# medivhna/TF_Face_Toolbox

Hardware: AMD Instinct MI355X
Metric: images/sec (whole node), SphereFaceNet-20 112x112 bs512 (higher is better)
Workload: dtype f32; 1 GPU; SphereFaceNet-20 + A-softmax training step, 112x112x3, global batch 512, 10575 classes, Momentum, fp32; global_batch=512, per_gpu_batch=512, parallelism=dp1

## Files before the change

### tf_face_toolbox_amd/csrc/api.hip

```cpp
#include <hip/hip_runtime.h>
#include <stdio.h>
#include <stdlib.h>
#include <string.h>

#include <initializer_list>

#include "../../include/fte.h"
#include "conv_plan.h"
#include "igemm.h"
#include "wgrad16.h"
#include "pw16.h"
#include "kernels.h"
#include "layers.h"
#include "wino.h"
#include "search.h"
#include "partial_fc.h"
#include "cluster.h"
#include "iresnet.h"

namespace {

inline int rc(hipError_t e) { return e == hipSuccess ? FTE_OK : (int)e; }

const PlanKnobs& knobs() {
    static const PlanKnobs k = plan_knobs_from_env();
    return k;
}
const Planner& planner(PlanCtx c, int epi) {
    if (c.bf16 || c.bn) {
        static const Planner host = {knobs(), {}};
        return host;
    }
    auto with_device = [](int e) {
        Planner p = {knobs(), {}};
        p.d.cus = igemm_num_cus();
        const int tile = sk_tile(p.k, e);
        for (int t : {tile, tile == TILE_128x128 ? (int)TILE_128x64 : tile})
            if (t >= 0 && t < 5) p.d.sk_bpc[t][e] = igemm_sk_blocks_per_cu(t, e);
        return p;
    };
    if (epi == EPI_FWD) {
        static const Planner fwd = with_device(EPI_FWD);
        return fwd;
    }
    static const Planner dgrad = with_device(EPI_DGRAD);
    return dgrad;
}
inline PlanCtx ctx32(bool bn = false) { return {igemm_get_bf16(), false, bn, wino_get_algo()}; }
inline PlanCtx ctx16(bool s16, bool bn = false) { return {true, s16, bn, wino_get_algo()}; }
template <class F>
size_t max_over_modes(bool bn, F total) {
    size_t need = 0;
    const int algo = wino_get_algo();
    for (const PlanCtx& c : {PlanCtx{false, false, bn, algo}, PlanCtx{true, false, bn, algo}, PlanCtx{true, true, bn, algo}}) {
        const size_t v = total(c);
        if (v > need) need = v;
    }
    return need;
}

inline void zero_params(IgemmParams* p) { memset(p, 0, sizeof(*p)); }

inline void plain_a(IgemmParams* p, const float* a, int ld, int kc) {
    p->A = a; p->a_OH = 1; p->a_OW = 1; p->a_IH = 1; p->a_IW = 1; p->a_stride = 1;
    p->a_ld = ld; p->a_KC = kc; p->a_NT = 1;
}
inline void conv_taps(IgemmParams* p, int ksize, const Pads& ph, const Pads& pw) {
    p->a_NT = ksize * ksize;
    for (int r = 0; r < ksize; ++r)
        for (int s = 0; s < ksize; ++s) { p->a_dh[r * ksize + s] = r - ph.before; p->a_dw[r * ksize + s] = s - pw.before; }
}

inline bool set_bytes(IgemmParams* p, size_t a_elems, size_t b_elems, size_t esize = 4) {
    const size_t lim = (size_t)1 << 31;
    if (a_elems * esize >= lim || b_elems * esize >= lim) return false;
    p->a_bytes = (unsigned)(a_elems * esize);
    p->b_bytes = (unsigned)(b_elems * esize);
    return true;
}

inline hipError_t launch_rows(IgemmParams p, const RowPlan& rp, int al, int bl, int epi, long prow0, float* pw, hipStream_t st) {
    const int M = p.M;
    hipError_t e = hipSuccess;
    if (rp.tail_mode == 3) {
        int bm, bn;
        igemm_tile_dims(rp.main_tile, &bm, &bn);
        const long T = rp.main_mtiles * (p.N / bn), iters = T * (p.K / 32);
        p.m_base = 0; p.prow0 = (int)prow0;
        p.sk_workers = rp.sk_workers; p.sk_base = (int)(iters / rp.sk_workers); p.sk_rem = (int)(iters % rp.sk_workers);
        p.SKW = pw; p.SKF = reinterpret_cast<unsigned*>(pw + (size_t)rp.sk_workers * bm * bn);
        return igemm_launch(p, al, bl, epi, rp.main_tile, 1, st);
    }
// ... 200 lines not shown
    a.x = x; a.w = w; a.bias = bias; a.alpha = alpha; a.res = res; a.z = z; a.y = y;
    a.vpack = vpack; a.xalpha = xalpha; a.z_only_ok = true;
    return a.run();
}
int fte_conv3x3_algo(int n, int h, int wd, int cin, int cout, int stride, int op) {
    if (op < 0 || op > 2) return FTE_EINVAL;
    return wino_wanted(knobs(), ctx32(), {n, h, wd, cin, cout, 3, stride}, op) ? FTE_CONV_WINOGRAD : FTE_CONV_DIRECT;
}
size_t fte_wino_pack_bytes(int n, int h, int wd, int c) {
    if (n <= 0 || h < 2 || wd < 2 || c <= 0 || c % 64) return 0;
    return wino_pack_floats(wino_geom(n, h, wd).M, c) * sizeof(float);
}

static size_t dgrad_ws_bytes(const ConvShape& s, bool bn) {
    if (s.n <= 0 || s.cin <= 0 || s.cin % 64 || s.cout % 32) return 0;
    return max_over_modes(bn, [&](PlanCtx c) { return dgrad_layout(planner(c, EPI_DGRAD), c, s).total; });
}
size_t fte_conv2d_dgrad_ws_bytes(int n, int h, int wd, int cin, int cout, int ksize, int stride) {
    return dgrad_ws_bytes({n, h, wd, cin, cout, ksize, stride}, false);
}

struct DgradBn {
    const void* zbn; const void* ybn;
    const float* gamma; const float* mean; const float* rstd; const float* scale; const float* shift;
    float* dgamma; float* dbeta; float* coef;
};
struct DgradArgs {
    PlanCtx ctx; ConvShape s; void* ws; size_t ws_bytes; void* stream;
    const void* dz; const void* w; bool src16; const float* addin; const float* zprev; const float* alpha_prev;
    float* raw; float* dzprev; uint16_t* dzprev16; float* dalpha_prev; float* dbias_prev;
    const uint16_t* addin16; const uint16_t* zprev16; uint16_t* raw16; const DgradBn* bn;
    int run();
};
int DgradArgs::run() {
    const int n = s.n, h = s.h, wd = s.wd, cin = s.cin, cout = s.cout, ksize = s.ksize, stride = s.stride;
    const float* zx = nullptr;
    const uint16_t* zx16 = nullptr;
    if (bn) {
        const void* msk = (!bn->scale && bn->ybn) ? bn->ybn : bn->zbn;
        const void* zb = (!bn->scale && bn->ybn) ? bn->zbn : nullptr;
        if (src16) { zprev16 = (const uint16_t*)msk; zx16 = (const uint16_t*)zb; }
        else { zprev = (const float*)msk; zx = (const float*)zb; }
        alpha_prev = bn->gamma;
        dalpha_prev = bn->dgamma; dbias_prev = bn->dbeta;
    }
    if (zprev16 && !zprev) zprev = reinterpret_cast<const float*>(zprev16);
    const bool z16only = zprev16 != nullptr;
    if (!dz || !w || (!dzprev && !(src16 && dzprev16)) || n <= 0 || cout % 32 || cin % 64 || (stride != 1 && stride != 2) || (ksize != 1 && ksize != 3)) return FTE_EINVAL;
    if (zprev && !alpha_prev) return FTE_EINVAL;
    const Pads pho = same_pads(h, ksize, stride), pwo = same_pads(wd, ksize, stride);
    const DgradLayout lay = dgrad_layout(planner(ctx, EPI_DGRAD), ctx, s);
    if (lay.wino && dzprev && !dzprev16 && !addin16 && !zprev16 && !raw16) {
        const WinoGeom g = wino_geom(n, h, wd);
        const size_t half_w = lay.wino_half;
        const WinoWs& wl = lay.w;
        if (ws && ws_bytes >= wl.total) {
            if (!aligned16({dz, w, addin, zprev, alpha_prev, raw, dzprev, ws})) return FTE_EINVAL;
            const bool part = zprev && (dalpha_prev || dbias_prev);
            float* V = (float*)((char*)ws + wl.v_off);
            float* U = (float*)((char*)ws + wl.u_off);
            hipError_t e = wino_transform_filter((const float*)w, U, cin, cout, 1, (hipStream_t)stream);
            if (e != hipSuccess) return (int)e;
            e = wino_transform_tiles((const float*)dz, V, n, h, wd, cout, 0, (hipStream_t)stream);
            if (e != hipSuccess) return (int)e;
            WinoMMParams q;
            memset(&q, 0, sizeof(q));
            q.V = V; q.U = U; q.K = cout; q.N = cin; q.g = g;
            q.ADD = addin; q.RAW = raw; q.Zin = zprev; q.alpha = alpha_prev; q.amod = cin; q.DZ = dzprev;
            q.PA = part ? (float*)ws : nullptr; q.PB = part ? (float*)((char*)ws + half_w) : nullptr;
            e = wino_mm(q, EPI_DGRAD, (hipStream_t)stream);
            if (e != hipSuccess) return (int)e;
            if (part) {
                float* scratch = (float*)((char*)ws + 2 * half_w);
                if (dalpha_prev && dbias_prev) return rc(k_reduce_rows2(q.PA, dalpha_prev, q.PB, dbias_prev, nullptr, 1, g.MB, cin, 1, 1.f, scratch, (hipStream_t)stream));
                if (dalpha_prev) return rc(k_reduce_rows(q.PA, dalpha_prev, nullptr, 1, g.MB, cin, 1, 1.f, scratch, (hipStream_t)stream));
                return rc(k_reduce_rows(q.PB, dbias_prev, nullptr, 1, g.MB, cin, 1, 1.f, scratch, (hipStream_t)stream));
            }
            return FTE_OK;
        }
    }
    const DgradClass* cls = lay.cls;
    const int nc = lay.nc;
    const bool merged = lay.merged;
    const long rows = lay.rows;
    const bool want_part = zprev && (dalpha_prev || dbias_prev);
    const size_t half = lay.half, pw_need = lay.pw_bytes;
    if ((want_part || pw_need) && (!ws || ws_bytes < lay.need)) return FTE_EWORKSPACE;
    float* scratch = want_part ? (float*)((char*)ws + lay.scratch_off) : nullptr;
    float* pwbuf = pw_need ? (float*)((char*)ws + lay.pw_off) : nullptr;
    float* PA = want_part ? (float*)ws : nullptr;
    float* PB = want_part ? (float*)((char*)ws + half) : nullptr;
    if (merged) {
        const int* order = lay.order;
        const int tile = lay.merged_tile;
        IgemmParams p;
        zero_params(&p);
        const DgradClass& c0 = cls[0];
        p.M = n * c0.hq * c0.wq; p.N = cin; p.a_KC = cout;
        p.A = (const float*)dz; p.a_OH = c0.hq; p.a_OW = c0.wq; p.a_IH = pho.out; p.a_IW = pwo.out; p.a_stride = 1; p.a_ld = cout;
        p.ncls = nc;
        int t = 0;
        for (int k = 0; k < nc; ++k) {
            const DgradClass& c = cls[order[k]];
            p.cls_tap0[k] = t; p.cls_ph[k] = c.ph; p.cls_pw[k] = c.pw;
            for (int j = 0; j < c.ntap; ++j, ++t) { p.a_dh[t] = c.dh[j]; p.a_dw[t] = c.dw[j]; p.b_tapoff[t] = c.wt[j] * cin * cout; }
        }
        p.cls_tap0[nc] = t;
        p.a_NT = t; p.K = t * cout; p.kchunk = p.K;
        p.B = (const float*)w; p.b_ld = cout;
        p.c_OH = c0.hq; p.c_OW = c0.wq; p.c_FH = h; p.c_FW = wd; p.c_step = stride; p.c_ld = cin;
        p.ADD = addin; p.RAW = raw; p.Zin = z16only ? nullptr : zprev; p.alpha = alpha_prev; p.amod = cin; p.DZ = dzprev;
        p.ADD16 = addin16; p.Zin16 = zprev16; p.RAW16 = raw16;
        p.PA = PA; p.PB = PB; p.prow0 = 0;
        if (bn) { p.bn_mu = bn->mean; p.bn_rs = bn->rstd; p.bn_sc = bn->scale; p.bn_sh = bn->shift; p.Zx = zx; p.Zx16 = zx16; }
        p.src16 = src16 ? 1 : 0; p.DZ16 = dzprev16;
        if (!set_bytes(&p, (size_t)n * pho.out * pwo.out * cout, (size_t)ksize * ksize * cin * cout, src16 ? 2 : 4)) return FTE_EINVAL;
        hipError_t e = igemm_launch(p, AL_MK, BL_NK, EPI_DGRAD, tile, 1, (hipStream_t)stream);
        if (e != hipSuccess) return (int)e;
    } else {
    long prow = 0;
    for (int i = 0; i < nc; ++i) {
        const DgradClass& c = cls[i];
        IgemmParams p;
        zero_params(&p);
        p.M = n * c.hq * c.wq; p.N = cin; p.K = c.ntap * cout; p.kchunk = p.K;
        p.A = (const float*)dz; p.a_OH = c.hq; p.a_OW = c.wq; p.a_IH = pho.out; p.a_IW = pwo.out; p.a_stride = 1;
        p.a_ld = cout; p.a_KC = cout; p.a_NT = c.ntap;
        for (int t = 0; t < c.ntap; ++t) {
            p.a_dh[t] = c.dh[t]; p.a_dw[t] = c.dw[t];
            p.b_tapoff[t] = c.wt[t] * cin * cout;
        }
        p.B = (const float*)w; p.b_ld = cout;
        p.src16 = src16 ? 1 : 0; p.DZ16 = dzprev16;
        if (stride == 1) { p.c_OH = 0; }
        else { p.c_OH = c.hq; p.c_OW = c.wq; p.c_FH = h; p.c_FW = wd; p.c_step = stride; p.c_ph = c.ph; p.c_pw = c.pw; }
        p.c_ld = cin;
        p.ADD = addin; p.RAW = raw; p.Zin = z16only ? nullptr : zprev; p.alpha = alpha_prev; p.amod = cin; p.DZ = dzprev;
        p.ADD16 = addin16; p.Zin16 = zprev16; p.RAW16 = raw16;
        p.PA = PA; p.PB = PB;
        if (bn) { p.bn_mu = bn->mean; p.bn_rs = bn->rstd; p.bn_sc = bn->scale; p.bn_sh = bn->shift; p.Zx = zx; p.Zx16 = zx16; }
        if (!set_bytes(&p, (size_t)n * pho.out * pwo.out * cout, (size_t)ksize * ksize * cin * cout, src16 ? 2 : 4)) return FTE_EINVAL;
        hipError_t e = launch_rows(p, c.rp, AL_MK, BL_NK, EPI_DGRAD, prow, pwbuf, (hipStream_t)stream);
        if (e != hipSuccess) return (int)e;
        prow += c.mtiles;
    }
    }
    if (bn)
        return rc(l_bn_bwd_finalize(PB, PA, cin, (int)rows, (long)n * h * wd, cin, bn->gamma, bn->mean, bn->rstd, bn->dgamma, bn->dbeta,
                                    bn->coef, (hipStream_t)stream));
    if (want_part) {
        if (dalpha_prev && dbias_prev) {
            hipError_t e = k_reduce_rows2(PA, dalpha_prev, PB, dbias_prev, nullptr, 1, rows, cin, 1, 1.f, scratch, (hipStream_t)stream);
            if (e != hipSuccess) return (int)e;
        } else {
            if (dalpha_prev) { hipError_t e = k_reduce_rows(PA, dalpha_prev, nullptr, 1, rows, cin, 1, 1.f, scratch, (hipStream_t)stream); if (e != hipSuccess) return (int)e; }
            if (dbias_prev) { hipError_t e = k_reduce_rows(PB, dbias_prev, nullptr, 1, rows, cin, 1, 1.f, scratch, (hipStream_t)stream); if (e != hipSuccess) return (int)e; }
        }
    }
    return FTE_OK;
}

int fte_conv2d_dgrad(const float* dz, const float* w, const float* addin, const float* zprev,
                     const float* alpha_prev, float* raw, float* dzprev, float* dalpha_prev, float* dbias_prev,
                     int n, int h, int wd, int cin, int cout, int ksize, int stride, void* ws, size_t ws_bytes, void* stream) {
    DgradArgs a = {ctx32(), {n, h, wd, cin, cout, ksize, stride}, ws, ws_bytes, stream};
    a.dz = dz; a.w = w;
    a.addin = addin; a.zprev = zprev; a.alpha_prev = alpha_prev; a.raw = raw; a.dzprev = dzprev; a.dalpha_prev = dalpha_prev; a.dbias_prev = dbias_prev;
    return a.run();
}
int fte_conv2d_dgrad16(const uint16_t* dz16, const uint16_t* w16, const float* addin, const float* zprev,
                       const float* alpha_prev, float* raw, float* dzprev, uint16_t* dzprev16, float* dalpha_prev, float* dbias_prev,
                       int n, int h, int wd, int cin, int cout, int ksize, int stride, void* ws, size_t ws_bytes, void* stream) {
    DgradArgs a = {ctx16(false), {n, h, wd, cin, cout, ksize, stride}, ws, ws_bytes, stream};
    a.dz = dz16; a.w = w16; a.src16 = true;
    a.addin = addin; a.zprev = zprev; a.alpha_prev = alpha_prev; a.raw = raw; a.dzprev = dzprev; a.dzprev16 = dzprev16;
// ... 1107 lines not shown
```

### tf_face_toolbox_amd/csrc/conv_plan.h

```cpp
#pragma once
#include <stddef.h>
#include <stdlib.h>
#include <string.h>

enum { EPI_FWD = 0, EPI_DGRAD = 1 };
enum { TILE_128x128 = 0, TILE_256x64 = 1, TILE_128x64 = 2, TILE_64x64 = 3, TILE_192x64 = 4,
       TILE_64x64_W1 = 5, TILE_64x64_W2 = 6 };
constexpr int FIXUP_CHUNKS = 4;
constexpr long REDUCE_SCRATCH_FLOATS = 1 << 18;

inline void igemm_tile_dims(int tile, int* bm, int* bn) {
    switch (tile) {
        case TILE_128x128: *bm = 128; *bn = 128; break;
        case TILE_256x64:  *bm = 256; *bn = 64; break;
        case TILE_128x64:  *bm = 128; *bn = 64; break;
        case TILE_192x64:  *bm = 192; *bn = 64; break;
        default:           *bm = 64;  *bn = 64; break;
    }
}
inline size_t igemm_sk_ws_bytes(int tile, int workers) {
    int bm, bn;
    igemm_tile_dims(tile, &bm, &bn);
    return (size_t)workers * bm * bn * sizeof(float) + (((size_t)workers * 4 + 255) & ~(size_t)255);
}

struct WinoGeom {
    int n, h, w, th, tw;
    long M;
    int MB;
};
inline WinoGeom wino_geom(int n, int h, int w) {
    WinoGeom g;
    g.n = n; g.h = h; g.w = w; g.th = (h + 1) / 2; g.tw = (w + 1) / 2;
    g.M = (long)n * g.th * g.tw;
    g.MB = (int)((g.M + 63) / 64);
    return g;
}
inline size_t wino_pack_floats(long rows, int c) { return (size_t)((rows + 63) / 64) * 64 * (size_t)c * 16; }
inline int wino_wgrad_splits(int cin, int cout) {
    if (cin % 64 || cout % 64) return 0;
    const int P = (cin / 64) * (cout / 64);
    if (P > 256 || 256 % P) return 0;
    return 256 / P;
}

struct PlanCtx {
    bool bf16;
    bool s16;
    bool bn;
    int algo;
};

struct PlanDevice {
    int cus;
    int sk_bpc[5][2];
};

struct PlanKnobs {
    long pick_want, pick_want16, fills16;
    int narrow_tile, wide_tile; bool narrow_tile_set, wide_tile_set;
    int sk, sk_tile, sk_tile_dgrad, sk_ops; double sk_max_per_cu; long sk_min_steps;
    bool plan_unsplit16, plan16_nosplit, tail_split_set;
    int min_splitp, split_minsteps, split_mink, split_rounds, split_minrounds;
    int wino_min_c, wino_fwd_tpb, wino_ops, wino_ops64;
    bool dgrad_cls_big, dgrad_merged16, dgrad_classes_set; char dgrad_classes;
    bool wgrad_split_major; int wgrad_tile;
};
inline PlanKnobs plan_knobs_from_env() {
    auto num = [](const char* name, long dflt) { const char* e = getenv(name); return e ? atol(e) : dflt; };
    auto flag = [](const char* name, int dflt) { const char* e = getenv(name); return e ? atoi(e) : dflt; };
    PlanKnobs k;
    memset(&k, 0, sizeof(k));
    k.pick_want = num("FTE_PICK_WANT", 384); k.pick_want16 = num("FTE_PICK_WANT16", 120); k.fills16 = num("FTE_FILLS16", 384);
    k.narrow_tile = flag("FTE_NARROW_TILE", TILE_64x64); k.narrow_tile_set = getenv("FTE_NARROW_TILE") != nullptr;
    k.wide_tile = flag("FTE_WIDE_TILE", TILE_64x64); k.wide_tile_set = getenv("FTE_WIDE_TILE") != nullptr;
    k.sk = flag("FTE_SK", 1);
    k.sk_tile = flag("FTE_SK_TILE", -1); k.sk_tile_dgrad = flag("FTE_SK_TILE_DGRAD", k.sk_tile);
    k.sk_ops = flag("FTE_SK_OPS", 3);
    k.sk_max_per_cu = getenv("FTE_SK_MAX_PER_CU") ? atof(getenv("FTE_SK_MAX_PER_CU")) : 4.0;
    k.sk_min_steps = num("FTE_SK_MIN_STEPS", 12);
    k.plan_unsplit16 = flag("FTE_PLAN_UNSPLIT16", 1) != 0; k.plan16_nosplit = flag("FTE_PLAN16_NOSPLIT", 1) != 0;
    k.tail_split_set = getenv("FTE_TAIL_SPLIT") != nullptr;
    k.min_splitp = flag("FTE_MIN_SPLITP", 2); k.split_minsteps = flag("FTE_SPLIT_MINSTEPS", 0);
    k.split_mink = flag("FTE_SPLIT_MINK", 256);
    k.split_rounds = flag("FTE_SPLIT_ROUNDS", 3); k.split_minrounds = flag("FTE_SPLIT_MINROUNDS", 1);
    k.wino_min_c = flag("FTE_WINO_MIN_C", 128); k.wino_fwd_tpb = flag("FTE_WINO_FWD_TPB", 256);
    k.wino_ops = flag("FTE_WINO_OPS", 7); k.wino_ops64 = flag("FTE_WINO_OPS64", 5);
    k.dgrad_cls_big = flag("FTE_DGRAD_CLS_BIG", 0) == 1; k.dgrad_merged16 = flag("FTE_DGRAD_MERGED16", 0) == 1;
    k.dgrad_classes_set = getenv("FTE_DGRAD_CLASSES") != nullptr; k.dgrad_classes = k.dgrad_classes_set ? getenv("FTE_DGRAD_CLASSES")[0] : 0;
    k.wgrad_split_major = flag("FTE_WGRAD_SPLIT_MAJOR", 1) != 0;
    k.wgrad_tile = flag("FTE_WGRAD_TILE", -1);
    return k;
}
struct Planner { PlanKnobs k; PlanDevice d; };

struct Pads { int out, before; };
inline Pads same_pads(int in, int k, int stride) {
    const int out = (in + stride - 1) / stride;
    int total = (out - 1) * stride + k - in;
    if (total < 0) total = 0;
    return {out, total / 2};
}
struct ConvShape { int n, h, wd, cin, cout, ksize, stride; };

inline size_t align_up(size_t v) { return (v + 255) & ~(size_t)255; }
constexpr size_t SCRATCH_BYTES = (size_t)REDUCE_SCRATCH_FLOATS * sizeof(float);

inline long tiles_of(int tile, long M, long N) {
    int bm, bn;
    igemm_tile_dims(tile, &bm, &bn);
    return ((M + bm - 1) / bm) * (N / bn);
}

inline int pick_tile(const PlanKnobs& k, bool bf16, long M, long N) {
    const long want = bf16 ? k.pick_want16 : k.pick_want;
    const int cands[3] = {N % 128 == 0 ? TILE_128x128 : TILE_256x64, TILE_128x64, TILE_64x64};
    for (int i = 0; i < 3; ++i)
        if (tiles_of(cands[i], M, N) >= want) return cands[i];
    return cands[2];
}

constexpr long SLOTS_BIG = 768;
constexpr long SLOTS = 1536;

struct RowPlan {
    int main_tile; long main_rows, main_mtiles;
    int tail_mode, tail_tile; long tail_mtiles; int tail_splits, tail_kchunk; size_t pw_bytes;
    int sk_workers;
};

inline int sk_tile(const PlanKnobs& k, int epi) {
    const int want = epi == EPI_FWD ? k.sk_tile : k.sk_tile_dgrad;
    return want >= 0 ? want : (epi == EPI_FWD ? TILE_64x64 : TILE_128x64);
}
inline bool plan_sk(const Planner& pl, long M, long N, long K, int epi, RowPlan* out) {
    const PlanKnobs& k = pl.k;
    if (!k.sk || K % 32 || N % 64 || !(k.sk_ops & (epi == EPI_FWD ? 1 : 2))) return false;
    const long ksteps = K / 32;
    int tile = sk_tile(k, epi);
    if (tile == TILE_128x128 && N % 128) tile = TILE_128x64;
    const int bpc = tile < 5 ? pl.d.sk_bpc[tile][epi] : 0;
    if (bpc <= 0) return false;
    int bm, bn;
    igemm_tile_dims(tile, &bm, &bn);
    const long MT = (M + bm - 1) / bm, T = MT * (N / bn), iters = T * ksteps;
    long W = (long)pl.d.cus * bpc;
    if (iters >= (1L << 31)) return false;
    if (k.sk == 1) {
        const double per_cu = (double)(((M + 127) / 128) * (N / 64)) / pl.d.cus;
        if (per_cu > k.sk_max_per_cu) return false;
        if (iters / W < k.sk_min_steps) return false;
    }
    if (W > iters) W = iters;
    memset(out, 0, sizeof(*out));
    out->main_tile = tile; out->main_rows = M; out->main_mtiles = MT;
    out->tail_mode = 3; out->sk_workers = (int)W;
    out->pw_bytes = igemm_sk_ws_bytes(tile, (int)W);
    return true;
}

inline RowPlan plan_rows(const Planner& pl, PlanCtx c, long M, long N, long K, bool allow_pw, bool small_only = false, int epi = -1) {
    const PlanKnobs& k = pl.k;
    RowPlan r;
    memset(&r, 0, sizeof(r));
    if (c.bn) allow_pw = false;
    if (epi >= 0 && allow_pw && !small_only && !c.bf16 && plan_sk(pl, M, N, K, epi, &r)) return r;
    const bool fills = ((M + 127) / 128) * (N / 128) >= k.fills16;
    const int wide = (!k.wide_tile_set && c.bf16 && !small_only && fills) ? TILE_128x128 : k.wide_tile;
    const bool fills_n = ((M + 127) / 128) * (N / 64) >= k.fills16;
    const int narrow = (!k.narrow_tile_set && c.bf16 && !small_only && fills_n) ? TILE_128x64 : k.narrow_tile;
    const bool tall = !k.wide_tile_set && !k.narrow_tile_set && !c.bf16 && !small_only && K >= 576 && ((M + 127) / 128) * (N / 64) >= 4096;
    const int big = tall ? TILE_128x64 : ((N % 128 == 0) ? wide : narrow);
    int bm, bn;
    igemm_tile_dims(big, &bm, &bn);
// ... 145 lines not shown
    int nc = 0;
    for (int a = 0; a < s.stride; ++a)
        for (int b = 0; b < s.stride; ++b) {
            DgradClass& c = cls[nc];
            c.ph = a; c.pw = b;
            c.hq = (s.h - a + s.stride - 1) / s.stride;
            c.wq = (s.wd - b + s.stride - 1) / s.stride;
            c.ntap = 0;
            if (c.hq <= 0 || c.wq <= 0) continue;
            for (int r = 0; r < s.ksize; ++r) {
                if ((a + ph.before - r) % s.stride) continue;
                for (int t = 0; t < s.ksize; ++t) {
                    if ((b + pw.before - t) % s.stride) continue;
                    c.dh[c.ntap] = (a + ph.before - r) / s.stride;
                    c.dw[c.ntap] = (b + pw.before - t) / s.stride;
                    c.wt[c.ntap] = r * s.ksize + t;
                    ++c.ntap;
                }
            }
            c.rp = plan_rows(pl, ctx, (long)s.n * c.hq * c.wq, s.cin, (long)c.ntap * s.cout, true, s.stride != 1 && !pl.k.dgrad_cls_big, EPI_DGRAD);
            c.mtiles = c.rp.main_mtiles + c.rp.tail_mtiles;
            ++nc;
        }
    return nc;
}
inline bool dgrad_mergeable(const PlanKnobs& k, PlanCtx c, const DgradClass* cls, int nc, int n, int cin) {
    if (nc != 4 || k.dgrad_classes == 's') return false;
    for (int i = 0; i < nc; ++i)
        if (cls[i].hq != cls[0].hq || cls[i].wq != cls[0].wq || cls[i].ntap < 1) return false;
    if (k.dgrad_classes == 'm' || (k.dgrad_merged16 && c.bf16)) return true;
    const long tiles = (((long)n * cls[0].hq * cls[0].wq + 63) / 64) * (cin / 64);
    return tiles < SLOTS;
}
inline int dgrad_merged_tile(const PlanKnobs& k, PlanCtx c, int cin) {
    if (!(k.dgrad_merged16 && c.bf16)) return TILE_64x64;
    return cin % 128 == 0 ? TILE_128x128 : TILE_128x64;
}
inline long dgrad_merged_rows(const PlanKnobs& k, PlanCtx c, const DgradClass* cls, int nc, int n, int cin) {
    if (!dgrad_mergeable(k, c, cls, nc, n, cin)) return 0;
    int bm, bn;
    igemm_tile_dims(dgrad_merged_tile(k, c, cin), &bm, &bn);
    return (long)nc * (((long)n * cls[0].hq * cls[0].wq + bm - 1) / bm);
}
inline int dgrad_merged_plan(const PlanKnobs& k, PlanCtx c, const DgradClass* cls, int nc, int cin, int* order) {
    for (int i = 0; i < nc; ++i) order[i] = i;
    for (int i = 0; i < nc; ++i)
        for (int j = i + 1; j < nc; ++j)
            if (cls[order[j]].ntap > cls[order[i]].ntap) { const int t = order[i]; order[i] = order[j]; order[j] = t; }
    return dgrad_merged_tile(k, c, cin);
}
struct DgradLayout {
    int nc; DgradClass cls[4];
    bool merged; int merged_tile, order[4];
    long rows;
    size_t half, scratch_off, pw_off, pw_bytes, need;
    bool wino; size_t wino_half; WinoWs w;
    size_t total;
};
inline DgradLayout dgrad_layout(const Planner& pl, PlanCtx c, const ConvShape& s) {
    DgradLayout l;
    memset(&l, 0, sizeof(l));
    l.nc = dgrad_classes(pl, c, s, l.cls);
    l.merged = dgrad_mergeable(pl.k, c, l.cls, l.nc, s.n, s.cin);
    long rows = 0;
    size_t pw = 0;
    for (int i = 0; i < l.nc; ++i) { rows += l.cls[i].mtiles; if (l.cls[i].rp.pw_bytes > pw) pw = l.cls[i].rp.pw_bytes; }
    const long merged_rows = dgrad_merged_rows(pl.k, c, l.cls, l.nc, s.n, s.cin);
    if (l.merged) l.merged_tile = dgrad_merged_plan(pl.k, c, l.cls, l.nc, s.cin, l.order);
    l.rows = l.merged ? merged_rows : rows;
    l.half = align_up((size_t)l.rows * s.cin * sizeof(float));
    l.scratch_off = 2 * l.half; l.pw_off = l.scratch_off + SCRATCH_BYTES;
    l.pw_bytes = l.merged ? 0 : pw;
    l.need = l.pw_off + l.pw_bytes;
    l.total = 2 * align_up((size_t)(merged_rows > rows ? merged_rows : rows) * s.cin * sizeof(float)) + SCRATCH_BYTES + pw;
    l.wino = wino_wanted(pl.k, c, s, 1);
    if (wino_sized(pl.k, c.algo, s, 1)) {
        l.wino_half = align_up((size_t)wino_geom(s.n, s.h, s.wd).MB * s.cin * sizeof(float));
        l.w = wino_ws(s, 1, 2 * l.wino_half + SCRATCH_BYTES);
        if (l.w.total > l.total) l.total = l.w.total;
    }
    return l;
}

inline void wgrad_plan(const PlanKnobs& k, const ConvShape& s, int* tile, int* splits, int* kchunk, int* K) {
    const Pads ph = same_pads(s.h, s.ksize, s.stride), pw = same_pads(s.wd, s.ksize, s.stride);
    *K = s.n * ph.out * pw.out;
    const long M = (long)s.ksize * s.ksize * s.cin;
    const int narrow = (M % 192 == 0 && M % 128 != 0) ? TILE_192x64 : TILE_128x64;
    const bool tiny = s.ksize == 1 && M * s.cout <= 256L * 256;
    *tile = k.wgrad_tile >= 0 ? k.wgrad_tile : (tiny ? TILE_64x64 : (s.cout % 128 == 0) ? TILE_128x128 : narrow);
    plan_splits(k, tiles_of(*tile, M, s.cout), *K, splits, kchunk, false);
    if (k.wgrad_tile < 0 && *tile != TILE_64x64 && *splits > 1 && *kchunk < 1024) {
        *tile = TILE_64x64;
        plan_splits(k, tiles_of(*tile, M, s.cout), *K, splits, kchunk, false);
    }
}
struct WgradLayout {
    int tile, splits, kchunk, K;
    size_t slab_bytes;
    bool wino; WinoWs w, w_kept;
    size_t total;
};
inline WgradLayout wgrad_layout(const PlanKnobs& k, PlanCtx c, const ConvShape& s, size_t resident3 = 0, size_t resident1 = 0) {
    WgradLayout l;
    memset(&l, 0, sizeof(l));
    wgrad_plan(k, s, &l.tile, &l.splits, &l.kchunk, &l.K);
    l.slab_bytes = l.splits > 1 ? (size_t)l.splits * s.ksize * s.ksize * s.cin * s.cout * sizeof(float) : 0;
    l.total = l.slab_bytes;
    if (resident3 > l.total) l.total = resident3;
    if (resident1 > l.total) l.total = resident1;
    l.wino = wino_wanted(k, c, s, 2);
    if (wino_sized(k, c.algo, s, 2)) {
        l.w = l.w_kept = wino_ws(s, 2, 0);
        const size_t vsz = l.w.u_off - l.w.v_off;
        l.w_kept.u_off -= vsz; l.w_kept.slab_off -= vsz; l.w_kept.total -= vsz;
        if (l.w.total > l.total) l.total = l.w.total;
    }
    l.total += SCRATCH_BYTES;
    return l;
}
```

Before: 15250 images/sec.

## Add fused single-kernel dgrad for 3x3 stride-2 convs covering all four parity classes

Adds a dedicated HIP kernel that computes the data gradient of 3x3 stride-2 convolutions for all four output parity classes in one pass. It reuses one shared dz tile in LDS with per-class shifted reads. The epilogue fuses residual add, PReLU backward and per-tile partial sums for alpha/bias gradients. This replaces the per-class or merged implicit-GEMM path plus its separate workspace handling. The kernel is enabled by default when the tile count is large enough, and it adds a new hand-scheduled MFMA kernel whose correctness and occupancy are unproven.

```diff
diff --git a/tf_face_toolbox_amd/csrc/api.hip b/tf_face_toolbox_amd/csrc/api.hip
--- a/tf_face_toolbox_amd/csrc/api.hip
+++ b/tf_face_toolbox_amd/csrc/api.hip
@@ -8,6 +8,7 @@
 #include "../../include/fte.h"
 #include "conv_plan.h"
 #include "igemm.h"
+#include "dgrad_s2.h"
 #include "wgrad16.h"
 #include "pw16.h"
 #include "kernels.h"
@@ -374,7 +375,7 @@
     const DgradClass* cls = lay.cls;
     const int nc = lay.nc;
     const bool merged = lay.merged;
-    const long rows = lay.rows;
+    long rows = lay.rows;
     const bool want_part = zprev && (dalpha_prev || dbias_prev);
     const size_t half = lay.half, pw_need = lay.pw_bytes;
     if ((want_part || pw_need) && (!ws || ws_bytes < lay.need)) return FTE_EWORKSPACE;
@@ -382,7 +383,21 @@
     float* pwbuf = pw_need ? (float*)((char*)ws + lay.pw_off) : nullptr;
     float* PA = want_part ? (float*)ws : nullptr;
     float* PB = want_part ? (float*)((char*)ws + half) : nullptr;
-    if (merged) {
+    bool fused = false;
+    if (!src16 && !bn && dzprev && !dzprev16 && !addin16 && !zprev16 && !raw16 && dgrad_s2_fused(knobs(), ctx, s)) {
+        DgradS2Params q;
+        memset(&q, 0, sizeof(q));
+        q.dz = (const float*)dz; q.w = (const float*)w; q.n = n; q.hq = h / 2; q.wq = wd / 2; q.cin = cin; q.cout = cout;
+        q.ADD = addin; q.RAW = raw; q.Zin = zprev; q.alpha = alpha_prev; q.DZ = dzprev; q.PA = PA; q.PB = PB;
+        if (dgrad_s2_handles(q)) {
+            hipError_t e = dgrad_s2_launch(q, (hipStream_t)stream);
+            if (e != hipSuccess) return (int)e;
+            fused = true;
+            rows = dgrad_s2_rows(s);
+        }
+    }
+    if (fused) {
+    } else if (merged) {
         const int* order = lay.order;
         const int tile = lay.merged_tile;
         IgemmParams p;
diff --git a/tf_face_toolbox_amd/csrc/conv_plan.h b/tf_face_toolbox_amd/csrc/conv_plan.h
--- a/tf_face_toolbox_amd/csrc/conv_plan.h
+++ b/tf_face_toolbox_amd/csrc/conv_plan.h
@@ -65,6 +65,7 @@
     int wino_min_c, wino_fwd_tpb, wino_ops, wino_ops64;
     bool dgrad_cls_big, dgrad_merged16, dgrad_classes_set; char dgrad_classes;
     bool wgrad_split_major; int wgrad_tile;
+    int dgrad_s2_fused;
 };
 inline PlanKnobs plan_knobs_from_env() {
     auto num = [](const char* name, long dflt) { const char* e = getenv(name); return e ? atol(e) : dflt; };
@@ -90,6 +91,7 @@
     k.dgrad_classes_set = getenv("FTE_DGRAD_CLASSES") != nullptr; k.dgrad_classes = k.dgrad_classes_set ? getenv("FTE_DGRAD_CLASSES")[0] : 0;
     k.wgrad_split_major = flag("FTE_WGRAD_SPLIT_MAJOR", 1) != 0;
     k.wgrad_tile = flag("FTE_WGRAD_TILE", -1);
+    { const char* e = getenv("FTE_DGRAD_S2_FUSED"); k.dgrad_s2_fused = (!e || e[0] == 'a') ? 2 : (atoi(e) != 0 ? 1 : 0); }
     return k;
 }
 struct Planner { PlanKnobs k; PlanDevice d; };
@@ -401,6 +403,21 @@
     return l;
 }
 
+constexpr long DGRAD_S2_MIN_TILES = 1024;
+constexpr int DGRAD_S2_BM = 64, DGRAD_S2_MAX_WQ = 31;
+inline bool dgrad_s2_shape_ok(const ConvShape& s) {
+    if (s.ksize != 3 || s.stride != 2 || s.n <= 0 || s.h < 2 || s.wd < 2 || (s.h & 1) || (s.wd & 1)) return false;
+    if (s.cin <= 0 || s.cout <= 0 || s.cin % 64 || s.cout % 32 || s.wd / 2 > DGRAD_S2_MAX_WQ) return false;
+    const size_t lim = (size_t)1 << 31, M = (size_t)s.n * (s.h / 2) * (s.wd / 2);
+    return M * s.cout * 4 < lim && 4 * M * s.cin * 4 < lim && (size_t)9 * s.cin * s.cout * 4 < lim;
+}
+inline long dgrad_s2_rows(const ConvShape& s) { return ((long)s.n * (s.h / 2) * (s.wd / 2) + DGRAD_S2_BM - 1) / DGRAD_S2_BM; }
+inline bool dgrad_s2_fused(const PlanKnobs& k, PlanCtx c, const ConvShape& s) {
+    if (c.bf16 || c.s16 || c.bn || c.algo == 0 || k.dgrad_s2_fused == 0 || !dgrad_s2_shape_ok(s)) return false;
+    if (k.dgrad_s2_fused == 1) return true;
+    return dgrad_s2_rows(s) * (s.cin / 64) >= DGRAD_S2_MIN_TILES;
+}
+
 inline void wgrad_plan(const PlanKnobs& k, const ConvShape& s, int* tile, int* splits, int* kchunk, int* K) {
     const Pads ph = same_pads(s.h, s.ksize, s.stride), pw = same_pads(s.wd, s.ksize, s.stride);
     *K = s.n * ph.out * pw.out;
diff --git a/tf_face_toolbox_amd/csrc/dgrad_s2.h b/tf_face_toolbox_amd/csrc/dgrad_s2.h
--- /dev/null
+++ b/tf_face_toolbox_amd/csrc/dgrad_s2.h
@@ -0,0 +1,12 @@
+#pragma once
+#include <hip/hip_runtime.h>
+
+struct DgradS2Params {
+    const float* dz;
+    const float* w;
+    int n, hq, wq, cin, cout;
+    const float* ADD; float* RAW; const float* Zin; const float* alpha; float* DZ; float* PA; float* PB;
+};
+
+bool dgrad_s2_handles(const DgradS2Params& p);
+hipError_t dgrad_s2_launch(const DgradS2Params& p, hipStream_t st);
diff --git a/tf_face_toolbox_amd/csrc/dgrad_s2.hip b/tf_face_toolbox_amd/csrc/dgrad_s2.hip
--- /dev/null
+++ b/tf_face_toolbox_amd/csrc/dgrad_s2.hip
@@ -0,0 +1,252 @@
+#include <hip/hip_runtime.h>
+#include <stdint.h>
+
+#include "dgrad_s2.h"
+#include "igemm.h"
+#include "igemm_dev.h"
+
+namespace {
+
+using namespace igemm_dev;
+
+constexpr int S2_BM = 64, S2_BN = 64, S2_LDR = 36;
+constexpr int S2_AROWS = 96;
+constexpr int S2_A_FLOATS = (S2_AROWS + 1) * S2_LDR, S2_B_FLOATS = S2_BN * S2_LDR;
+constexpr size_t S2_LDS_LOOP = (size_t)(S2_A_FLOATS + S2_B_FLOATS) * sizeof(float);
+constexpr size_t S2_LDS_EPI = (size_t)(S2_BM + 4 * 32 * 36 + 2 * 2 * S2_BN) * sizeof(float);
+constexpr size_t S2_LDS = S2_LDS_LOOP > S2_LDS_EPI ? S2_LDS_LOOP : S2_LDS_EPI;
+
+typedef const __attribute__((address_space(3))) f32x4* lds_cf4;
+typedef __attribute__((address_space(3))) f32x4* lds_f4;
+
+__global__ __launch_bounds__(256, 4) void dgrad_s2_kernel(const DgradS2Params p) {
+    extern __shared__ __attribute__((aligned(16))) float smem[];
+    const int tid = threadIdx.x;
+    const int lane = tid & 63, wid = tid >> 6;
+    const int wm = wid >> 1, wn = wid & 1;
+    const int li = lane & 31, lh = lane >> 5;
+    __builtin_amdgcn_s_setprio(3);
+
+    const int M = p.n * p.hq * p.wq, ntn = p.cin / S2_BN, H = p.wq + 1;
+    int bid = blockIdx.x;
+    {
+        const int ntiles = gridDim.x;
+        const int q = ntiles >> 3, r = ntiles & 7, xcd = bid & 7, loc = bid >> 3;
+        bid = (xcd < r ? xcd * (q + 1) : r * (q + 1) + (xcd - r) * q) + loc;
+    }
+    const int mt = bid / ntn, nt_ = bid - mt * ntn;
+    const int m0 = mt * S2_BM, n0 = nt_ * S2_BN;
+
+    constexpr unsigned OOB = 0x80000000u;
+    const unsigned a_bytes = (unsigned)M * (unsigned)p.cout * 4u, b_bytes = 9u * (unsigned)p.cin * (unsigned)p.cout * 4u;
+    const __amdgpu_buffer_rsrc_t rsrcA = __builtin_amdgcn_make_buffer_rsrc(const_cast<float*>(p.dz), 0, a_bytes, 0x00020000);
+    const __amdgpu_buffer_rsrc_t rsrcB = __builtin_amdgcn_make_buffer_rsrc(const_cast<float*>(p.w), 0, b_bytes, 0x00020000);
+    auto ldg = [&](const __amdgpu_buffer_rsrc_t& r, unsigned voff, unsigned soff) -> f32x4 {
+        return __builtin_bit_cast(f32x4, __builtin_amdgcn_raw_buffer_load_b128(r, voff, soff, 0));
+    };
+
+    unsigned a_off[3], b_off[2];
+#pragma unroll
+    for (int i = 0; i < 3; ++i) {
+        const int j = (tid >> 3) + 32 * i, g = m0 - H + j;
+        const bool ok = g >= 0 && g < M && j < H + S2_BM;
+        a_off[i] = ok ? ((unsigned)g * (unsigned)p.cout + (unsigned)((tid & 7) << 2)) * 4u : OOB;
+    }
+#pragma unroll
+    for (int j = 0; j < 2; ++j)
+        b_off[j] = ((unsigned)(n0 + (tid >> 3) + 32 * j) * (unsigned)p.cout + (unsigned)((tid & 7) << 2)) * 4u;
+    __attribute__((address_space(3))) char* const lbase = (__attribute__((address_space(3))) char*)smem;
+    const unsigned ldsB = (unsigned)S2_A_FLOATS * 4u;
+    unsigned a_wr[3], b_wr[2];
+#pragma unroll
+    for (int i = 0; i < 3; ++i) a_wr[i] = (unsigned)((((tid >> 3) + 32 * i) * S2_LDR + ((tid & 7) << 2)) * 4);
+#pragma unroll
+    for (int j = 0; j < 2; ++j) b_wr[j] = ldsB + (unsigned)((((tid >> 3) + 32 * j) * S2_LDR + ((tid & 7) << 2)) * 4);
+
+    unsigned a_rd[4];
+    {
+        const int r = wm * 32 + li, m = m0 + r;
+        const int hw = p.hq * p.wq;
+        const int rem = m - (m / hw) * hw;
+        const int q = rem / p.wq, pc = rem - q * p.wq;
+#pragma unroll
+        for (int s = 0; s < 4; ++s) {
+            const int sft = ((s & 2) ? p.wq : 0) + (s & 1);
+            const bool valid = !((s & 2) && q == 0) && !((s & 1) && pc == 0);
+            a_rd[s] = (unsigned)((valid ? (r + H - sft) * S2_LDR + 4 * lh : S2_AROWS * S2_LDR) * 4);
+        }
+    }
+    const unsigned b_rd = ldsB + (unsigned)(((wn * 32 + li) * S2_LDR + 4 * lh) * 4);
+    auto lds_ld = [&](unsigned off) -> f32x4 { return *(lds_cf4)(lbase + off); };
+    auto lds_st = [&](unsigned off, const f32x4& v) { *(lds_f4)(lbase + off) = v; };
+
+    f32x16 acc[4];
+#pragma unroll
+    for (int c = 0; c < 4; ++c)
+#pragma unroll
+        for (int r = 0; r < 16; ++r) acc[c][r] = 0.f;
+
+    f32x4 ra[3], rb[2];
+    const int nch = p.cout / BK;
+    const unsigned tapstride = (unsigned)p.cin * (unsigned)p.cout;
+#pragma unroll
+    for (int i = 0; i < 3; ++i) ra[i] = ldg(rsrcA, a_off[i], 0);
+#pragma unroll
+    for (int j = 0; j < 2; ++j) rb[j] = ldg(rsrcB, b_off[j], 0);
+    if (tid < S2_LDR) smem[S2_AROWS * S2_LDR + tid] = 0.f;
+#pragma unroll
+    for (int i = 0; i < 3; ++i) lds_st(a_wr[i], ra[i]);
+#pragma unroll
+    for (int j = 0; j < 2; ++j) lds_st(b_wr[j], rb[j]);
+    __syncthreads();
+    __builtin_amdgcn_s_setprio(0);
+
+    for (int g = 0; g < nch; ++g) {
+        const int gn = g + 1 < nch ? g + 1 : g;
+        const unsigned a_soff = (unsigned)(gn * BK) * 4u;
+        static_for<0, 9>([&](auto tc) {
+            constexpr int T = decltype(tc)::value, R = T / 3, S = T % 3;
+            constexpr int CLS = (R & 1) * 2 + (S & 1), SH = (R == 2 ? 2 : 0) + (S == 2 ? 1 : 0);
+            constexpr int TNX = (T + 1) % 9;
+            const unsigned b_soff = ((unsigned)TNX * tapstride + (unsigned)((T == 8 ? gn : g) * BK)) * 4u;
+            f32x4 fa0 = lds_ld(a_rd[SH]), fb0 = lds_ld(b_rd);
+            f32x4 fa1 = lds_ld(a_rd[SH] + 32u), fb1 = lds_ld(b_rd + 32u);
+            __builtin_amdgcn_sched_barrier(0);
+            static_for<0, 16>([&](auto ic) {
+                constexpr int idx = decltype(ic)::value, u = idx / 4, t = idx % 4;
+                if constexpr ((u & 1) == 0)
+                    acc[CLS] = __builtin_amdgcn_mfma_f32_32x32x2f32(fa0[t], fb0[t], acc[CLS], 0, 0, 0);
+                else
+                    acc[CLS] = __builtin_amdgcn_mfma_f32_32x32x2f32(fa1[t], fb1[t], acc[CLS], 0, 0, 0);
+                if constexpr (idx < 2) rb[idx] = ldg(rsrcB, b_off[idx], b_soff);
+                if constexpr (T == 7 && idx >= 2 && idx < 5) ra[idx - 2] = ldg(rsrcA, a_off[idx - 2], a_soff);
+                if constexpr (idx == 4) { fa0 = lds_ld(a_rd[SH] + 64u); fb0 = lds_ld(b_rd + 64u); }
+                if constexpr (idx == 8) { fa1 = lds_ld(a_rd[SH] + 96u); fb1 = lds_ld(b_rd + 96u); }
+                if constexpr (idx == 12) __syncthreads();
+                if constexpr (T == 8 && idx == 13) {
+#pragma unroll
+                    for (int i = 0; i < 3; ++i) lds_st(a_wr[i], ra[i]);
+                }
+                if constexpr (idx >= 14) lds_st(b_wr[idx - 14], rb[idx - 14]);
+                __builtin_amdgcn_sched_barrier(0);
+            });
+            __syncthreads();
+        });
+    }
+
+    __builtin_amdgcn_s_setprio(2);
+    int* rowoff = reinterpret_cast<int*>(smem);
+    const int FW = 2 * p.wq;
+    for (int r = tid; r < S2_BM; r += 256) {
+        const int m = m0 + r;
+        int off = -1;
+        if (m < M) {
+            const int hw = p.hq * p.wq;
+            const int ni = m / hw, rem = m - ni * hw;
+            const int q = rem / p.wq, pc = rem - q * p.wq;
+            off = ((ni * 2 * p.hq + 2 * q) * FW + 2 * pc) * p.cin;
+        }
+        rowoff[r] = off;
+    }
+    __syncthreads();
+    float* patch = smem + S2_BM + wid * (32 * 36);
+    const int prw = lane >> 3, pc4 = lane & 7;
+    const int col = n0 + wn * 32 + 4 * pc4;
+    const bool act = p.Zin != nullptr;
+    f32x4 al4 = {1.f, 1.f, 1.f, 1.f};
+    if (act) {
+#pragma unroll
+        for (int e = 0; e < 4; ++e) al4[e] = p.alpha[col + e];
+    }
+    f32x4 sa4 = {0.f, 0.f, 0.f, 0.f}, sb4 = {0.f, 0.f, 0.f, 0.f};
+    int offs[4];
+#pragma unroll
+    for (int ps = 0; ps < 4; ++ps) offs[ps] = rowoff[wm * 32 + prw + 8 * ps];
+    static_for<0, 4>([&](auto cc) {
+        constexpr int CLS = decltype(cc)::value;
+        const int coff = ((CLS >> 1) * FW + (CLS & 1)) * p.cin;
+        f32x4 in0[4], in1[4];
+#pragma unroll
+        for (int ps = 0; ps < 4; ++ps) {
+            const long o = (long)(offs[ps] < 0 ? 0 : offs[ps] + coff) + col;
+            in0[ps] = f32x4{0.f, 0.f, 0.f, 0.f};
+            in1[ps] = f32x4{0.f, 0.f, 0.f, 0.f};
+            if (p.ADD && offs[ps] >= 0) in0[ps] = *reinterpret_cast<const f32x4*>(p.ADD + o);
+            if (p.Zin && offs[ps] >= 0) in1[ps] = *reinterpret_cast<const f32x4*>(p.Zin + o);
+        }
+        __builtin_amdgcn_wave_barrier();
+#pragma unroll
+        for (int r = 0; r < 16; ++r) patch[((r & 3) + 8 * (r >> 2) + 4 * lh) * 36 + li] = acc[CLS][r];
+        __builtin_amdgcn_fence(__ATOMIC_RELEASE, "wavefront");
+        __builtin_amdgcn_wave_barrier();
+#pragma unroll
+        for (int ps = 0; ps < 4; ++ps) {
+            f32x4 v = *reinterpret_cast<const f32x4*>(patch + (prw + 8 * ps) * 36 + 4 * pc4);
+            if (offs[ps] < 0) continue;
+            const long o = (long)(offs[ps] + coff) + col;
+            v += in0[ps];
+            if (p.RAW) *reinterpret_cast<f32x4*>(p.RAW + o) = v;
+            if (act) {
+                const f32x4 z = in1[ps];
+#pragma unroll
+                for (int e = 0; e < 4; ++e) {
+                    sa4[e] += v[e] * fminf(z[e], 0.f);
+                    v[e] *= prelu_slope(z[e], al4[e]);
+                    sb4[e] += v[e];
+                }
+            }
+            *reinterpret_cast<f32x4*>(p.DZ + o) = v;
+        }
+    });
+    if (p.PA) {
+        __syncthreads();
+        float* red = smem + S2_BM + 4 * (32 * 36);
+#pragma unroll
+        for (int e = 0; e < 4; ++e) {
+            float a = sa4[e], b = sb4[e];
+            a += __shfl_xor(a, 8); b += __shfl_xor(b, 8);
+            a += __shfl_xor(a, 16); b += __shfl_xor(b, 16);
+            a += __shfl_xor(a, 32); b += __shfl_xor(b, 32);
+            if (prw == 0) {
+                const int c = wn * 32 + 4 * pc4 + e;
+                red[wm * S2_BN + c] = a;
+                red[(2 + wm) * S2_BN + c] = b;
+            }
+        }
+        __syncthreads();
+        for (int c = tid; c < S2_BN; c += 256) {
+            const float a = red[c] + red[S2_BN + c], b = red[2 * S2_BN + c] + red[3 * S2_BN + c];
+            const long o = (long)mt * p.cin + n0 + c;
+            p.PA[o] = a;
+            if (p.PB) p.PB[o] = b;
+        }
+    }
+}
+
+}
+
+bool dgrad_s2_handles(const DgradS2Params& p) {
+    if (!p.dz || !p.w || !p.DZ || p.n <= 0 || p.hq <= 0 || p.wq <= 0 || p.wq + 1 + S2_BM > S2_AROWS) return false;
+    if (p.cin <= 0 || p.cout <= 0 || p.cin % S2_BN || p.cout % 32) return false;
+    const size_t lim = (size_t)1 << 31;
+    const size_t M = (size_t)p.n * p.hq * p.wq;
+    if (M * p.cout * 4 >= lim || (size_t)9 * p.cin * p.cout * 4 >= lim || 4 * M * p.cin * 4 >= lim) return false;
+    const uintptr_t ptrs = (uintptr_t)p.dz | (uintptr_t)p.w | (uintptr_t)p.ADD | (uintptr_t)p.RAW | (uintptr_t)p.Zin | (uintptr_t)p.DZ;
+    if ((ptrs & 15) || (p.Zin && !p.alpha)) return false;
+    return true;
+}
+
+hipError_t dgrad_s2_launch(const DgradS2Params& p, hipStream_t st) {
+    if (!dgrad_s2_handles(p)) return hipErrorInvalidValue;
+    const long M = (long)p.n * p.hq * p.wq;
+    const long tiles = (M + S2_BM - 1) / S2_BM * (p.cin / S2_BN);
+    if (tiles >= (1L << 31)) return hipErrorInvalidValue;
+    const int sig[5] = {AL_MK, BL_NK, EPI_DGRAD, TILE_64x64, 1};
+    const double out = 4.0 * (double)M * p.cin * 4.0;
+    const double bytes = (double)M * p.cout * 4.0 + 9.0 * p.cin * p.cout * 4.0 + out * (1 + (p.ADD ? 1 : 0) + (p.Zin ? 1 : 0) + (p.RAW ? 1 : 0));
+    const int h = igemm_prof_begin(sig, (int)(4 * M), p.cin, 9 * p.cout / 4, 2.0 * 4.0 * (double)M * p.cin * (9.0 / 4.0) * p.cout, bytes, st);
+    hipLaunchKernelGGL(dgrad_s2_kernel, dim3((unsigned)tiles), dim3(256), S2_LDS, st, p);
+    const hipError_t e = hipGetLastError();
+    igemm_prof_end(h, "dgrad_s2_kernel", st);
+    return e;
+}
```

After: 15190 images/sec, median of 3. No clear change (-0.3%).
